# ekzhu/datasketch

Measured on AMD Instinct MI355X. Metric: MinHash signatures/sec (1M sets x 256 tokens, num_perm=128), higher is better.
Workload: dtype u64

## Files before the change

### datasketch_amd/csrc/mhx_api.hip

```cpp
#include <algorithm>
#include <cmath>
#include <condition_variable>
#include <cstdlib>
#include <cstring>
#include <mutex>
#include <new>
#include <system_error>
#include <thread>
#include <vector>

#include "mhx_internal.h"

namespace mhx {

static thread_local std::string g_last_error;

void set_error(const char *fmt, ...) {
    char buf[1024];
    va_list ap;
    va_start(ap, fmt);
    vsnprintf(buf, sizeof(buf), fmt, ap);
    va_end(ap);
    g_last_error = buf;
}
// ... 385 lines not shown
    MHX_ENTER(ctx, ctx);
    if (name && name_len > 0) {
        strncpy(name, ctx->name, (size_t)name_len - 1);
        name[name_len - 1] = 0;
    }
    if (cus) *cus = ctx->hw_cus;
    if (hbm_bytes) *hbm_bytes = ctx->hbm_bytes;
    return MHX_OK;
}

int mhx_ctx_set_option(mhx_ctx *ctx, const char *key, int64_t value) {
    static const struct {
        const char *key;
        int64_t mhx_ctx::*field;
    } options[] = {
        {"minhash.path", &mhx_ctx::opt_minhash_path},       {"minhash.split", &mhx_ctx::opt_minhash_split},
        {"minhash.packed", &mhx_ctx::opt_minhash_packed},   {"minhash.ties", &mhx_ctx::opt_minhash_ties},
        {"minhash.p3", &mhx_ctx::opt_minhash_p3},           {"minhash.share", &mhx_ctx::opt_minhash_share},
        {"minhash.adapt", &mhx_ctx::opt_minhash_adapt},     {"blocks_per_cu", &mhx_ctx::opt_blocks_per_cu},
        {"minhash.alias", &mhx_ctx::opt_minhash_alias},     {"minhash.prefetch", &mhx_ctx::opt_minhash_prefetch},
        {"weighted.path", &mhx_ctx::opt_weighted_path},     {"weighted.direct", &mhx_ctx::opt_weighted_direct},
        {"weighted.split", &mhx_ctx::opt_weighted_split},   {"weighted.tail", &mhx_ctx::opt_weighted_tail},
        {"weighted.debug", &mhx_ctx::opt_weighted_debug},   {"weighted.kernel", &mhx_ctx::opt_weighted_kernel},
        {"weighted.plan", &mhx_ctx::opt_weighted_plan},     {"weighted.rescue", &mhx_ctx::opt_weighted_rescue},
        {"weighted.min_dim", &mhx_ctx::opt_weighted_min_dim}, {"host.chunk_bytes", &mhx_ctx::opt_host_chunk_bytes},
        {"lsh.sort_bits", &mhx_ctx::opt_lsh_sort_bits},     {"lsh.gather", &mhx_ctx::opt_lsh_gather},
        {"lsh.sort", &mhx_ctx::opt_lsh_sort},               {"lsh.levels", &mhx_ctx::opt_lsh_levels},
        {"lsh.chunk", &mhx_ctx::opt_lsh_chunk},             {"lsh.team", &mhx_ctx::opt_lsh_team},
        {"lsh.bigbins", &mhx_ctx::opt_lsh_bigbins},         {"pack.fused", &mhx_ctx::opt_pack_fused},
        {"weighted.refill", &mhx_ctx::opt_weighted_refill}, {"lsh.prehash", &mhx_ctx::opt_lsh_prehash},
        {"lsh.merge_items", &mhx_ctx::opt_lsh_merge_items}, {"hll.split_tokens", &mhx_ctx::opt_hll_split_tokens},
        {"bloom.lanes", &mhx_ctx::opt_bloom_lanes},         {"jaccard.topk_path", &mhx_ctx::opt_jaccard_topk_path},
        {"jaccard.topk_segments", &mhx_ctx::opt_jaccard_topk_segments}, {"debug.cus", &mhx_ctx::opt_debug_cus},
    };
    if (!ctx || !key) return fail(MHX_ERR_INVALID, "ctx/key is NULL");
    MHX_GUARD(ctx);
    for (const auto &o : options) {
        if (strcmp(key, o.key)) continue;
        if (o.field == &mhx_ctx::opt_lsh_merge_items)
            MHX_REQUIRE(value == 0 || value == 8 || value == 16, "lsh.merge_items must be 0, 8 or 16");
        if (o.field == &mhx_ctx::opt_hll_split_tokens) MHX_REQUIRE(value >= 0, "hll.split_tokens must be >= 0");
        if (o.field == &mhx_ctx::opt_bloom_lanes) MHX_REQUIRE(value == 0 || value == 1 || value == 16, "bloom.lanes must be 0, 1 or 16");
        if (o.field == &mhx_ctx::opt_jaccard_topk_path) MHX_REQUIRE(value >= 0 && value <= 2, "jaccard.topk_path must be 0, 1 or 2");
        if (o.field == &mhx_ctx::opt_jaccard_topk_segments) MHX_REQUIRE(value >= 0, "jaccard.topk_segments must be >= 0");
        if (o.field == &mhx_ctx::opt_debug_cus)
            MHX_REQUIRE(value >= 0 && value <= ctx->hw_cus, "debug.cus must be 0 (the device's %d CUs) or in [1, %d], got %lld", ctx->hw_cus, ctx->hw_cus,
                        (long long)value);
        ctx->*o.field = value;
        if (o.field == &mhx_ctx::opt_debug_cus) ctx->num_cus = value ? (int)value : ctx->hw_cus;
        return MHX_OK;
    }
    return fail(MHX_ERR_INVALID, "unknown option '%s'", key);
}

int mhx_ctx_minhash_mode(mhx_ctx *ctx, int reset, int *mode) {
    MHX_ENTER(ctx, ctx);
    MHX_TRY(ctx->activate());
    MHX_TRY(ctx->ensure_work());
    unsigned int word = 0;
    MHX_HIP_CHECK(hipMemcpyAsync(&word, ctx->d_work + 8, sizeof(word), hipMemcpyDeviceToHost, ctx->stream));
    MHX_HIP_CHECK(hipStreamSynchronize(ctx->stream));
    if (mode) *mode = (int)word;
    if (reset) MHX_HIP_CHECK(hipMemsetAsync(ctx->d_work + 8, 0, sizeof(word), ctx->stream));
    return MHX_OK;
}

int mhx_ctx_minhash_flags(mhx_ctx *ctx, int64_t n_sets, uint8_t *flags) {
    MHX_ENTER(ctx, ctx);
    MHX_TRY(ctx->activate());
    MHX_REQUIRE(n_sets >= 0 && (flags || n_sets == 0), "NULL flags");
    if (ctx->redo_sets != n_sets || (n_sets > 0 && !ctx->d_redo))
        return fail(MHX_ERR_INVALID, "the last MinHash call on this context kept flags for %lld sets, not %lld (one huge set split over waves and "
                    "minhash.path != 0 keep none)", (long long)ctx->redo_sets, (long long)n_sets);
    MHX_HIP_CHECK(hipStreamSynchronize(ctx->stream));
    if (n_sets > 0) MHX_HIP_CHECK(hipMemcpy(flags, ctx->d_redo, (size_t)n_sets, hipMemcpyDeviceToHost));
    return MHX_OK;
}

int mhx_ctx_counters(mhx_ctx *ctx, int enable, uint64_t out[MHX_NUM_COUNTERS]) {
    MHX_ENTER(ctx, ctx);
    MHX_TRY(ctx->activate());
    MHX_HIP_CHECK(hipStreamSynchronize(ctx->stream));
    if (out) {
        for (int i = 0; i < MHX_NUM_COUNTERS; ++i) out[i] = 0;
        if (ctx->d_stats)
            MHX_HIP_CHECK(hipMemcpy(out, ctx->d_stats, sizeof(uint64_t) * MHX_NUM_COUNTERS, hipMemcpyDeviceToHost));
    }
    if (enable && !ctx->d_stats) {
        hipError_t e = mhx::dev_malloc(reinterpret_cast<void **>(&ctx->d_stats), sizeof(uint64_t) * MHX_NUM_COUNTERS);
        if (e != hipSuccess) {
            ctx->d_stats = nullptr;
            return fail(MHX_ERR_OOM, "counter allocation failed: %s", hipGetErrorString(e));
        }
    }
    if (!enable && ctx->d_stats) {
        MHX_HIP_CHECK(mhx::dev_free(ctx->d_stats));
        ctx->d_stats = nullptr;
    }
    if (ctx->d_stats) MHX_HIP_CHECK(hipMemset(ctx->d_stats, 0, sizeof(uint64_t) * MHX_NUM_COUNTERS));
    return MHX_OK;
}

int mhx_debug_guard_alloc(int align, int64_t *granule, int64_t *live) {
    if (align != 0 && (align < -4096 || align > 4096 || ((align < 0 ? -align : align) & ((align < 0 ? -align : align) - 1))))
        return fail(MHX_ERR_INVALID, "guard alignment must be 0 (off) or +-(a power of two <= 4096), got %d", align);
    (void)mhx::guard_mode();
    {
        std::lock_guard<std::mutex> lk(mhx::g_guard_mu);
// ... 1963 lines not shown
```

### datasketch_amd/csrc/mhx_internal.h

```cpp
#pragma once

#include <hip/hip_runtime.h>

#include <algorithm>
#include <cstdarg>
#include <cstdint>
#include <cstdio>
#include <mutex>
#include <string>
#include <unordered_map>

#include "mhx.h"

namespace mhx {

void set_error(const char *fmt, ...);
int fail(int code, const char *fmt, ...);
void forgive();

#define MHX_HIP_CHECK(expr)                                                                      \
    do {                                                                                         \
        hipError_t _e = (expr);                                                                  \
        if (_e != hipSuccess) {                                                                  \
            return ::mhx::fail(_e == hipErrorOutOfMemory ? MHX_ERR_OOM : MHX_ERR_HIP,            \
// ... 8 lines not shown
constexpr unsigned int kPairListCap = 16384;
constexpr size_t kWorkBytes = 64 + sizeof(unsigned int) * kPairListCap;

#define MHX_GUARD(ctxp) std::lock_guard<std::recursive_mutex> _mhx_guard((ctxp)->mu)

#define MHX_REQUIRE(cond, ...)                                       \
    do {                                                             \
        if (!(cond)) return ::mhx::fail(MHX_ERR_INVALID, __VA_ARGS__); \
    } while (0)

hipError_t dev_malloc(void **p, size_t bytes, bool caller = false);
hipError_t dev_free(void *p);
bool guard_mode();

}

struct mhx_ctx {
    std::recursive_mutex mu;
    int device = 0;
    hipStream_t stream = nullptr;
    int num_cus = 0;
    int hw_cus = 0;
    int64_t lds_per_block = 64 << 10;
    int64_t hbm_bytes = 0;
    char name[128] = {0};
    void *scratch[5] = {nullptr, nullptr, nullptr, nullptr, nullptr};
    size_t scratch_bytes[5] = {0, 0, 0, 0, 0};
    int64_t opt_minhash_path = 0;
    int64_t opt_minhash_packed = 0;
    int64_t opt_minhash_adapt = 0;
    int64_t opt_minhash_share = 0;
    int64_t opt_minhash_p3 = 0;
    int64_t opt_minhash_ties = 0;
    int64_t opt_minhash_split = 0;
    int64_t opt_blocks_per_cu = 0;
    int64_t opt_debug_cus = 0;
    int64_t opt_minhash_prefetch = 1;
    int64_t opt_minhash_alias = -1;
    int64_t opt_weighted_path = 0;
    int64_t opt_weighted_min_dim = 0;
    int64_t opt_weighted_rescue = 0;
    int64_t opt_weighted_plan = 0;
    int64_t opt_weighted_kernel = 0;
    int64_t opt_weighted_debug = 0;
    int64_t opt_weighted_split = 0;
    int64_t opt_weighted_tail = 0;
    int64_t opt_weighted_direct = 0;
    int64_t opt_lsh_sort = 0;
    int64_t opt_lsh_gather = 0;
    int64_t opt_lsh_sort_bits = 0;
    int64_t opt_lsh_prehash = 0;
    int64_t opt_lsh_chunk = 0;
    int64_t opt_lsh_bigbins = 0;
    int64_t opt_lsh_team = 0;
    int64_t opt_lsh_merge_items = 0;
    int64_t opt_lsh_levels = 0;
    int64_t opt_pack_fused = 0;
    int64_t opt_weighted_refill = 0;
    int64_t opt_hll_split_tokens = 0;
    int64_t opt_bloom_lanes = 0;
    int64_t opt_jaccard_topk_path = 0;
    int64_t opt_jaccard_topk_segments = 0;
    int64_t opt_host_chunk_bytes = 0;

    hipStream_t copy_in = nullptr;
    hipStream_t copy_out = nullptr;
// ... 144 lines not shown
```

### datasketch_amd/csrc/minhash_kernels.hip

```cpp
#include <type_traits>

#include "mhx_internal.h"

namespace mhx {
namespace {

constexpr uint64_t kMersenne = (1ull << 61) - 1;
constexpr uint32_t kMaxHash = 0xFFFFFFFFu;
constexpr int kWave = 64;

struct BulkArgs {
    const void *hv;
    const int64_t *offsets;
    int64_t fixed_len;
    int64_t n_sets;
    const uint64_t *a;
    const uint64_t *b;
    int32_t num_perm;
    int32_t path;
    unsigned long long *stats;
    uint8_t *redo;
    int32_t redo_match;
    unsigned int *sieve_hint;
    unsigned int *mode_word;
// ... 237 lines not shown
    }
    __device__ __forceinline__ void merge_from_lane(int other) {
        const uint32_t o1 = (uint32_t)__shfl((int)k1, other, kWave), o2 = (uint32_t)__shfl((int)k2, other, kWave);
        const uint32_t o3 = (uint32_t)__shfl((int)k3, other, kWave);
        add(o1);
        add(o2);
        add(o3);
    }
};

template <int P, typename TokT, bool OPEN, int PS = P>
__device__ __forceinline__ void sieve_chunk(const Chunk<TokT> &c, const SievePerms<P> &sp, uint32_t (&row)[P]) {
    constexpr int N = Chunk<TokT>::N;
    c.keep_whole();
#pragma unroll
    for (int i = 0; i < N; i += 4) {
#pragma unroll
        for (int p = 0; p < PS; ++p) {
            const uint32_t m0 = sieve_key(c.lo(i + 0), sp.a_lo[p], sp.b8[p]);
            const uint32_t m1 = sieve_key(c.lo(i + 1), sp.a_lo[p], sp.b8[p]);
            const uint32_t m2 = sieve_key(c.lo(i + 2), sp.a_lo[p], sp.b8[p]);
            const uint32_t m3 = sieve_key(c.lo(i + 3), sp.a_lo[p], sp.b8[p]);
            row[p] = (OPEN && i == 0) ? min(m0, m1) : umin3(row[p], m0, m1);
            row[p] = umin3(row[p], m2, m3);
        }
        if constexpr (PS == 1)
            asm volatile("" : "+v"(row[0]));
        else
            asm volatile("" : "+v"(row[0]), "+v"(row[PS - 1]));
        __builtin_amdgcn_sched_barrier(0);
    }
}

template <int P, int STRIDE, int WPT, bool PARTIAL = false>
__device__ __forceinline__ bool finish_block(const Two (&rows)[P], const uint32_t *tile, const Perms<P> &pm,
                                             const SievePerms<P> &sp, uint32_t (&res)[P], uint32_t last_row = 16,
                                             uint32_t last_cols = 16) {
    Two cols[P];
    uint64_t best[P];
#pragma unroll
    for (int q = 0; q < P; ++q) {
        const uint32_t myrow = rows[q].k1 & 15u;
        const uint32_t *rowp = tile + myrow * STRIDE;
        const uint32_t limit = PARTIAL ? (myrow == last_row ? last_cols : 16u) : 16u;
        if constexpr (P <= 2) {
            uint32_t w[kRowTokens];
#pragma unroll
            for (int c = 0; c < kRowTokens; ++c) w[c] = rowp[c * WPT];
            const auto key = [&](int c) {
                uint32_t m = sieve_key(w[c], sp.a_lo[q], sp.b8[q]);
                if (PARTIAL) m = (uint32_t)c < limit ? m : kMaxHash;
                return tag16(m, (uint32_t)c);
            };
            uint32_t lo[5], mid[5];
#pragma unroll
            for (int i = 0; i < 5; ++i) {
                const uint32_t x = key(3 * i), y = key(3 * i + 1), z = key(3 * i + 2);
                lo[i] = umin3(x, y, z);
                mid[i] = umed3(x, y, z);
                asm volatile("" : "+v"(lo[i]), "+v"(mid[i]));
                __builtin_amdgcn_sched_barrier(0);
            }
            const uint32_t last = key(15);
            const uint32_t a1 = umin3(lo[0], lo[1], lo[2]), a2 = umed3(lo[0], lo[1], lo[2]);
            const uint32_t b1 = umin3(lo[3], lo[4], last), b2 = umed3(lo[3], lo[4], last);
            cols[q].k1 = min(a1, b1);
            cols[q].k2 = min(umin3(max(a1, b1), a2, b2), umin3(umin3(mid[0], mid[1], mid[2]), mid[3], mid[4]));
            asm volatile("" : "+v"(cols[q].k2));
        } else {
#pragma unroll
            for (int c = 0; c < kRowTokens; ++c) {
                uint32_t m = (uint32_t)((uint64_t)rowp[c * WPT] * sp.a_lo[q] + sp.b8[q]);
                if (PARTIAL) m = (uint32_t)c < limit ? m : kMaxHash;
                cols[q].add(tag16(m, (uint32_t)c));
            }
        }
        const uint32_t j1 = cols[q].k1 & 15u;
        best[q] = WPT == 2 ? *reinterpret_cast<const uint64_t *>(rowp + 2 * j1) : (uint64_t)rowp[j1];
        __builtin_amdgcn_sched_barrier(0);
    }
    bool fail = false;
#pragma unroll
    for (int q = 0; q < P; ++q) {
        const bool ok = rows[q].apart() && cols[q].apart() && cols[q].k1 >= 16u;
        fail |= sp.active[q] && !ok;
        uint32_t l0, h0;
        mad_wide((uint32_t)best[q], (uint32_t)(best[q] >> 32), pm.a_lo[q], pm.a_hi[q], pm.b[q], l0, h0);
        res[q] = min(res[q], fold_exact(l0, h0));
    }
    return fail;
}

template <int P, int STRIDE, int WPT>
__device__ __forceinline__ bool finish_block_ties(const Three (&rows)[P], const uint32_t *tile, const Perms<P> &pm,
                                                  const SievePerms<P> &sp, uint32_t (&res)[P], bool *tied = nullptr) {
    bool fail = false;
#pragma unroll
    for (int q = 0; q < P; ++q) {
        const uint32_t base = rows[q].k1 & ~15u;
        const uint32_t *rowp = tile + (rows[q].k1 & 15u) * STRIDE;
        Three cols;
#pragma unroll
        for (int c = 0; c < kRowTokens; ++c) {
            const uint32_t m = (uint32_t)((uint64_t)rowp[c * WPT] * sp.a_lo[q] + sp.b8[q]);
            cols.add(tag16(m, (uint32_t)c));
        }
        const bool row_tie = rows[q].k2 - base < 32u;
        const bool col_tie = cols.k2 - base < 32u;
        bool ok = base >= 16u && base <= 0xFFFFFF00u && rows[q].k3 - base >= 32u && !(row_tie && col_tie) && cols.k3 - base >= 32u;
        const uint32_t j1 = cols.k1 & 15u;
        const uint64_t t1 = WPT == 2 ? *reinterpret_cast<const uint64_t *>(rowp + 2 * j1) : (uint64_t)rowp[j1];
        const uint32_t j2 = col_tie ? (cols.k2 & 15u) : j1;
        uint64_t t2 = WPT == 2 ? *reinterpret_cast<const uint64_t *>(rowp + 2 * j2) : (uint64_t)rowp[j2];
        if (__any(row_tie)) {
            const uint32_t *row2 = tile + (rows[q].k2 & 15u) * STRIDE;
            Two other;
#pragma unroll
            for (int c = 0; c < kRowTokens; ++c) {
                const uint32_t m = (uint32_t)((uint64_t)row2[c * WPT] * sp.a_lo[q] + sp.b8[q]);
                other.add(tag16(m, (uint32_t)c));
            }
// ... 8 lines not shown
        if (tied) *tied |= sp.active[q] && (row_tie || col_tie);
        uint32_t l0, h0, l1, h1;
        mad_wide((uint32_t)t1, (uint32_t)(t1 >> 32), pm.a_lo[q], pm.a_hi[q], pm.b[q], l0, h0);
        mad_wide((uint32_t)t2, (uint32_t)(t2 >> 32), pm.a_lo[q], pm.a_hi[q], pm.b[q], l1, h1);
        res[q] = umin3(res[q], fold_exact(l0, h0), fold_exact(l1, h1));
        __builtin_amdgcn_sched_barrier(0);
    }
    return fail;
}

template <int P, int STRIDE, int WPT, typename Rows>
__device__ __forceinline__ void share_last_slot(Rows &rec, const uint32_t *tile, const SievePerms<P> &sp, int rb, int lane) {
    const uint32_t span = sp.span, groups = (uint32_t)kWave / span;
    const uint32_t mine = (uint32_t)lane / span;
    const uint32_t a_lo = sp.a_lo[P - 1];
    const uint64_t b8 = sp.b8[P - 1];
    rec = Rows();
#pragma unroll 1
    for (uint32_t r0 = 0; r0 < (uint32_t)rb; r0 += groups) {
        const uint32_t r = r0 + mine;
        const uint32_t *rowp = tile + (r & 15u) * STRIDE;
        uint32_t m = kMaxHash;
#pragma unroll
        for (int c = 0; c < kRowTokens; c += 2) {
            const uint32_t m0 = sieve_key(rowp[c * WPT], a_lo, b8);
            const uint32_t m1 = sieve_key(rowp[(c + 1) * WPT], a_lo, b8);
            m = umin3(m, m0, m1);
        }
        rec.add(r < (uint32_t)rb ? tag16(m, r) : kMaxHash);
    }
    for (uint32_t s = span; s < (uint32_t)kWave; s <<= 1) rec.merge_from_lane(lane ^ (int)s);
}

template <int P, typename TokT, bool TIES = false, bool SHARE = false>
__device__ __forceinline__ bool sieve_range(const TokT MHX_CONST_AS *hv, const TokT *hv_vec, int64_t beg,
                                            int nrows, const Perms<P> &pm, const SievePerms<P> &sp,
                                            uint32_t *lds, int lane, uint32_t (&res)[P], int &nblocks, bool *tied = nullptr) {
    constexpr int N = Chunk<TokT>::N;
    constexpr int CPR = kRowTokens / N;
    constexpr int STRIDE = StageLayout<TokT>::kStride, WPT = StageLayout<TokT>::kWordsPerTok;
    const TokT MHX_CONST_AS *p = hv + beg;
    const int nchunks = nrows * CPR;
    const auto chunk_ptr = [&](int idx) { return p + (int64_t)(idx < nchunks ? idx : nchunks - 1) * N; };
    Chunk<TokT> a, b;
    a.load(p);
    int ci = 0;
    bool fail = false;
    for (int r0 = 0; r0 < nrows; r0 += kBlockRows) {
        const int rb = min(kBlockRows, nrows - r0);
        const int64_t blk = beg + (int64_t)r0 * kRowTokens;
        const int my_row = lane >> 2, my_part = lane & 3;
        uint4 st0 = {0, 0, 0, 0}, st1 = {0, 0, 0, 0};
        if (my_row < rb) {
            const uint4 *src = reinterpret_cast<const uint4 *>(hv_vec + blk + 4 * lane);
            st0 = src[0];
            if (WPT == 2) st1 = src[1];
        }
        typename std::conditional<TIES, Three, Two>::type rows[P];
        const auto row_loop = [&](auto slots) {
            constexpr int PS = decltype(slots)::value;
            if constexpr (CPR == 2) {
                for (int r = 0; r < rb; ++r) {
                    uint32_t row0[P];
                    a.arrived();
                    b.load(chunk_ptr(ci + 1));
                    __builtin_amdgcn_sched_barrier(0);
                    sieve_chunk<P, TokT, true, PS>(a, sp, row0);
                    b.arrived();
                    a.load(chunk_ptr(ci + 2));
                    __builtin_amdgcn_sched_barrier(0);
// ... 5 lines not shown
            } else {
                for (int r = 0; r < rb; r += 2) {
                    uint32_t row0[P], row1[P];
                    a.arrived();
                    b.load(chunk_ptr(ci + 1));
                    __builtin_amdgcn_sched_barrier(0);
                    sieve_chunk<P, TokT, true, PS>(a, sp, row0);
                    b.arrived();
                    a.load(chunk_ptr(ci + 2));
                    __builtin_amdgcn_sched_barrier(0);
                    sieve_chunk<P, TokT, true, PS>(b, sp, row1);
                    ci += 2;
                    const bool second = r + 1 < rb;
                    if (!second) ci -= 1;
#pragma unroll
                    for (int q = 0; q < PS; ++q) {
                        rows[q].add(tag16(row0[q], (uint32_t)r));
                        if (second) rows[q].add(tag16(row1[q], (uint32_t)(r + 1)));
                    }
                }
            }
        };
        constexpr bool kShare = SHARE && P >= 3;
        row_loop(std::integral_constant<int, (kShare ? P - 1 : P)>());
        {
            uint4 *dst = reinterpret_cast<uint4 *>(lds + my_row * STRIDE + my_part * (4 * WPT));
            dst[0] = st0;
            if (WPT == 2) dst[1] = st1;
        }
        if constexpr (kShare) share_last_slot<P, STRIDE, WPT>(rows[P - 1], lds, sp, rb, lane);
        if constexpr (TIES)
            fail |= finish_block_ties<P, STRIDE, WPT>(rows, lds, pm, sp, res, tied);
        else
            fail |= finish_block<P, STRIDE, WPT>(rows, lds, pm, sp, res);
        ++nblocks;
    }
    return fail;
}

constexpr int kDedupSlots = 1024;
constexpr int kDedupPasses = 3;
constexpr int kDedupWordsPerWave = kStageWordsPerWave + kDedupSlots;

template <typename TokT>
__device__ __forceinline__ void load_quad(const TokT *hv_vec, int64_t blk, int64_t end, int lane, uint64_t (&t)[4]) {
#pragma unroll
    for (int i = 0; i < 4; ++i) t[i] = blk + 4 * lane + i < end ? (uint64_t)hv_vec[blk + 4 * lane + i] : 0;
}

template <int P, typename TokT>
__device__ __forceinline__ bool dedup_sieve_range(const TokT *hv_vec, int64_t beg, int64_t end, const Perms<P> &pm,
                                                  const SievePerms<P> &sp, uint32_t *lds, int lane,
                                                  const uint64_t (&first)[4], uint32_t (&res)[P]) {
    constexpr int STRIDE = 36;
    uint32_t *tile = lds;
    uint32_t *table = lds + kStageWordsPerWave;
    bool fail = false;
    for (int64_t blk = beg; blk < end; blk += kBlockRows * kRowTokens) {
        const int nb = (int)min((int64_t)(kBlockRows * kRowTokens), end - blk);
        uint64_t t[4];
        bool keep[4];
        if (blk == beg) {
#pragma unroll
            for (int i = 0; i < 4; ++i) t[i] = first[i];
        } else {
            load_quad<TokT>(hv_vec, blk, end, lane, t);
        }
// ... 110 lines not shown
    for (int p = 0; p < P; ++p) {
        const int k = kbase + p * kWave + lane;
        active[p] = k < num_perm;
        const uint64_t av = active[p] ? a[k] : 0;
        pm.a_lo[p] = pm_biased.a_lo[p] = (uint32_t)av;
        pm.a_hi[p] = pm_biased.a_hi[p] = (uint32_t)(av >> 32);
        pm.b[p] = active[p] ? b[k] : 0;
        pm_biased.b[p] = pm.b[p] + 1;
    }
    Minima<P> res;
    bool redo = exact_only;
    if (!exact_only) {
        uint32_t acc[P];
#pragma unroll
        for (int p = 0; p < P; ++p) acc[p] = kMaxHash;
        hash_range<P, false, TokT>(hv, beg, end, pm_biased, acc);
        bool suspicious = false;
#pragma unroll
        for (int p = 0; p < P; ++p) {
            suspicious |= active[p] && acc[p] <= 7u;
            res.v[p] = acc[p] - 1u;
        }
        redo = __any(suspicious);
    }
    if (redo) {
        if (!exact_only && stats && lane == 0) atomicAdd(stats + 1, 1ull);
#pragma unroll
        for (int p = 0; p < P; ++p) res.v[p] = kMaxHash;
        hash_range<P, true, TokT>(hv, beg, end, pm, res.v);
    }
    return res;
}

template <int P, typename TokT, bool TAIL = true, bool TIES = false, bool SHARE = false>
__device__ __forceinline__ bool sieve_minima(const TokT MHX_CONST_AS *hv, const TokT *hv_vec, int64_t beg,
                                             int64_t end, const Perms<P> &pm, const Perms<P> &pm_biased,
                                             const SievePerms<P> &sp, unsigned long long *stats, int lane,
                                             uint32_t *lds, uint32_t (&res)[P], bool *tied = nullptr) {
    const int64_t n = end - beg;
    const int nrows = (int)min(n / kRowTokens, (int64_t)(1 << 27));
#pragma unroll
    for (int p = 0; p < P; ++p) res[p] = kMaxHash;
    bool bad = false;
    if (nrows > 0) {
        int nblocks = 0;
        bad = sieve_range<P, TokT, TIES, SHARE>(hv, hv_vec, beg, nrows, pm, sp, lds, lane, res, nblocks, tied);
        if (stats && lane == 0) atomicAdd(stats + 2, (unsigned long long)nblocks);
    }
    const int64_t tail = beg + (int64_t)nrows * kRowTokens;
    if (TAIL && tail < end) {
        uint32_t acc[P];
#pragma unroll
        for (int p = 0; p < P; ++p) acc[p] = kMaxHash;
        hash_range<P, false, TokT>(hv, tail, end, pm_biased, acc);
#pragma unroll
        for (int p = 0; p < P; ++p) {
            bad |= sp.active[p] && acc[p] <= 7u;
            res[p] = min(res[p], acc[p] - 1u);
        }
    }
    return __any(bad);
}

struct SieveBackoff {
    int skip = 0;
    int gap = 16;
    int streak = 0;
    __device__ __forceinline__ void failed() {
        if (++streak >= 2) {
            skip = gap;
            gap = min(2 * gap, 64);
        }
    }
    __device__ __forceinline__ void succeeded() {
        streak = 0;
        gap = 16;
    }
};

// ... 38 lines not shown
    }
}

template <int P, bool SHARE = false>
__device__ __forceinline__ void load_perms(const BulkArgs &args, int kbase, int lane, Perms<P> &pm,
                                           Perms<P> &pm_biased, SievePerms<P> &sp, int (&kidx)[P]) {
    uint32_t span = kWave;
    if constexpr (SHARE && P >= 3) {
        const int r = args.num_perm - (kbase + (P - 1) * kWave);
        span = r > 16 ? 32u : r > 8 ? 16u : r > 4 ? 8u : 4u;
    }
    sp.span = span;
#pragma unroll
    for (int p = 0; p < P; ++p) {
        const bool shared = SHARE && P >= 3 && p == P - 1;
        const int k = kbase + p * kWave + (shared ? lane & (int)(span - 1) : lane);
        const bool holds = k < args.num_perm;
        kidx[p] = holds && !(shared && lane >= (int)span) ? k : -1;
        const uint64_t a = holds ? args.a[k] : 0;
        pm.a_lo[p] = (uint32_t)a;
        pm.a_hi[p] = (uint32_t)(a >> 32);
        pm.b[p] = holds ? args.b[k] : 0;
        pm_biased.a_lo[p] = pm.a_lo[p];
        pm_biased.a_hi[p] = pm.a_hi[p];
        pm_biased.b[p] = pm.b[p] + 1;
        sp.a_lo[p] = pm.a_lo[p];
        sp.b8[p] = pm.b[p] + 8;
        sp.active[p] = kidx[p] >= 0;
    }
}

enum { MODE_SIEVE = 0, MODE_FULL = 1, MODE_DEDUP = 2, MODE_SIEVE_TIES = 3 };
enum { SHAPE_GENERAL = 0, SHAPE_PLAIN = 1, SHAPE_PLAIN_FIXED = 2, SHAPE_PLAIN_FIXED_ROWS = 3 };

template <int P, typename TokT, typename OutT, int MODE, int SHAPE, bool SHARE = false>
__global__ __launch_bounds__(256) void minhash_bulk_kernel(const BulkArgs args_in) {
    BulkArgs args = args_in;
    constexpr bool kSieve = MODE == MODE_SIEVE || MODE == MODE_SIEVE_TIES;
    if (kSieve && args.mode_word) {
        const unsigned int want_ties = *as_const(args.mode_word);
        if ((want_ties == 1u) != (MODE == MODE_SIEVE_TIES)) return;
    }
    if (MODE == MODE_FULL && args.mode_word && args.sieve_hint && blockIdx.x == 0 && threadIdx.x == 0) {
        const unsigned int t = __builtin_nontemporal_load(args.sieve_hint), f = __builtin_nontemporal_load(args.sieve_hint + 1);
        const unsigned int g = __builtin_nontemporal_load(args.sieve_hint + 2), m = *args.mode_word;
        const unsigned int tt = __builtin_nontemporal_load(args.sieve_hint + 3), tf = __builtin_nontemporal_load(args.sieve_hint + 5);
        if (t >= 64u) {
            const bool defeated = 4u * f > t;
            const bool heavy = m == 1u ? 5u * g > t : (tt >= 64u ? 5u * tf > tt : m == 2u);
            *args.mode_word = !defeated ? 0u : heavy ? 2u : 1u;
        }
    }
    if (SHAPE != SHAPE_GENERAL) {
        args.init = nullptr;
        args.init_stride = 0;
        args.stats = nullptr;
        args.alias_mask = -1;
    }
    if (SHAPE == SHAPE_PLAIN_FIXED || SHAPE == SHAPE_PLAIN_FIXED_ROWS) args.offsets = nullptr;
    const int lane = threadIdx.x & (kWave - 1);
    const int wave = __builtin_amdgcn_readfirstlane(threadIdx.x >> 6);
    const int waves_per_block = blockDim.x >> 6;
    const int kchunks = (args.num_perm + kWave * P - 1) / (kWave * P);
    constexpr int kLdsPerWave = MODE == MODE_DEDUP ? kDedupWordsPerWave : kStageWordsPerWave;
    __shared__ __attribute__((aligned(16))) uint32_t stage[4 * kLdsPerWave];
    uint32_t *lds = stage + wave * kLdsPerWave;
    Perms<P> pm, pm_biased;
    SievePerms<P> sp;
    int kidx[P];
    if (kSieve || MODE == MODE_DEDUP) load_perms<P, SHARE>(args, 0, lane, pm, pm_biased, sp, kidx);

    const TokT MHX_CONST_AS *hv = as_const(static_cast<const TokT *>(args.hv));
    const TokT *hv_vec = static_cast<const TokT *>(args.hv);
    const int64_t MHX_CONST_AS *offsets = as_const(args.offsets);
    OutT *__restrict__ out = static_cast<OutT *>(args.out);
    const int64_t stride = (int64_t)gridDim.x * waves_per_block;
    const bool flagged_only = !kSieve && args.redo != nullptr;
    unsigned int listed_n = 0;
    bool listed = false;
    if (MODE == MODE_FULL && flagged_only && args.pair_list) {
        listed_n = *as_const(args.pair_count);
        listed = listed_n <= kPairListCap;
    }
    const int64_t n_items = listed ? (int64_t)listed_n : flagged_only ? (args.n_sets + kWave - 1) / kWave * waves_per_block : args.n_sets;
    SieveBackoff backoff;
    TiesBackoff ties;
    int tried = 0, failed = 0, left = 0;
    if (MODE == MODE_SIEVE && args.sieve_hint) {
        const unsigned int t = __builtin_nontemporal_load(args.sieve_hint), f = __builtin_nontemporal_load(args.sieve_hint + 1);
        if (t >= 64u && 2u * f > t) {
            backoff.skip = 63;
            backoff.gap = 64;
            backoff.streak = 2;
        }
    }
    if (MODE == MODE_FULL && listed) {
        uint32_t *comb = stage;
        for (int64_t it = blockIdx.x; it < (int64_t)listed_n; it += gridDim.x) {
            const int64_t set = (int64_t)as_const(args.pair_list)[it];
            const int64_t beg = args.offsets ? offsets[set] : set * args.fixed_len;
            const int64_t end = args.offsets ? offsets[set + 1] : beg + args.fixed_len;
            const int64_t share = (end - beg + 31) / 32 * 8;
            const int64_t wbeg = min(end, beg + wave * share), wend = min(end, wbeg + share);
            for (int kc = 0; kc < kchunks; ++kc) {
                uint32_t mine[P];
#pragma unroll
                for (int p = 0; p < P; ++p) mine[p] = kMaxHash;
                if (wend > wbeg) {
                    const Minima<P> m = full_minima<P, TokT>(hv_vec, wbeg, wend, args.a, args.b, args.num_perm, kc * (kWave * P),
                                                             args.path == 1, args.stats);
#pragma unroll
                    for (int p = 0; p < P; ++p) mine[p] = m.v[p];
                }
#pragma unroll
                for (int p = 0; p < P; ++p) comb[(wave * P + p) * kWave + lane] = mine[p];
                __syncthreads();
                if (wave == 0) {
#pragma unroll
                    for (int p = 0; p < P; ++p) {
                        const int k = kc * (kWave * P) + p * kWave + lane;
                        if (k >= args.num_perm) continue;
                        uint32_t r = mine[p];
// ... 27 lines not shown
        const int64_t set = listed ? (int64_t)as_const(args.pair_list)[item0] : flagged_only ? item * kWave + bit : item;
        int64_t beg, end;
        if (args.offsets) {
            beg = offsets[set];
            end = offsets[set + 1];
        } else {
            beg = (args.alias_mask >= 0 ? (set & args.alias_mask) : set) * args.fixed_len;
            end = beg + args.fixed_len;
        }
        uint32_t warm = 0;
        {
            const int64_t nset = listed ? args.n_sets : flagged_only ? (todo ? item * kWave + __builtin_ctzll(todo) : args.n_sets) : item + stride;
            const bool skipping_on = MODE == MODE_SIEVE && backoff.skip > 1;
            if (args.prefetch && nset < args.n_sets && !skipping_on) {
                const int64_t nbeg = args.offsets ? offsets[nset] : nset * args.fixed_len;
                const int64_t nend = args.offsets ? offsets[nset + 1] : nbeg + args.fixed_len;
                const int64_t off = (int64_t)lane * 128;
                if (off < (nend - nbeg) * (int64_t)sizeof(TokT))
                    warm = *reinterpret_cast<const volatile uint32_t *>(reinterpret_cast<const char *>(args.hv) +
                                                                         nbeg * (int64_t)sizeof(TokT) + off);
            }
        }
        bool defer = false;
        if (MODE == MODE_SIEVE && end > beg && backoff.skip > 0) {
            --backoff.skip;
            defer = true;
        }
        for (int kc = 0; kc < kchunks && !defer; ++kc) {
            uint32_t res[P];
            if (kSieve) {
                if (kchunks > 1) load_perms<P, SHARE>(args, kc * (kWave * P), lane, pm, pm_biased, sp, kidx);
                if (end > beg) {
                    bool tied = false;
                    defer = sieve_minima<P, TokT, SHAPE != SHAPE_PLAIN_FIXED_ROWS, MODE == MODE_SIEVE_TIES, SHARE>(hv, hv_vec, beg, end, pm, pm_biased, sp, args.stats, lane, lds, res,
                                                                                                          MODE == MODE_SIEVE_TIES ? &tied : nullptr);
                    if (kc == 0) ++tried;
                    if (MODE == MODE_SIEVE_TIES) {
                        if (defer || __any(tied)) ++failed;
                        if (defer) {
                            ++left;
                            break;
                        }
                    } else {
                        if (defer) {
                            ++failed;
                            backoff.failed();
                            break;
                        }
                        backoff.succeeded();
                    }
                }
            } else {
#pragma unroll
                for (int p = 0; p < P; ++p) {
                    const int k = kc * (kWave * P) + p * kWave + lane;
                    kidx[p] = k < args.num_perm ? k : -1;
                }
                if (end > beg) {
                    if (MODE == MODE_DEDUP) {
                        if (kchunks > 1) load_perms<P>(args, kc * (kWave * P), lane, pm, pm_biased, sp, kidx);
                        bool open = true;
                        if (!args.ties || (args.mode_word && *as_const(args.mode_word) == 1u)) {
                        } else if (ties.skip > 0) {
                            if (kc == kchunks - 1) --ties.skip;
                        } else {
                            open = sieve_minima<P, TokT, true, true>(hv, hv_vec, beg, end, pm, pm_biased, sp, nullptr, lane, lds, res);
                            if (kc == 0) ++tried, failed += open ? 1 : 0;
                            if (open) ties.failed(); else ties.succeeded();
                        }
                        if (open) {
#pragma unroll
                        for (int p = 0; p < P; ++p) res[p] = kMaxHash;
                        uint64_t cur[4];
                        load_quad<TokT>(hv_vec, beg, end, lane, cur);
                        defer = __any(dedup_sieve_range<P, TokT>(hv_vec, beg, end, pm, sp, lds, lane, cur, res));
                        if (defer) {
                            if (args.stats && lane == 0) atomicAdd(args.stats + 3, 1ull);
                            break;
                        }
                        }
                    } else {
                        const Minima<P> m = full_minima<P, TokT>(hv_vec, beg, end, args.a, args.b, args.num_perm,
                                                                 kc * (kWave * P), args.path == 1, args.stats);
#pragma unroll
                        for (int p = 0; p < P; ++p) res[p] = m.v[p];
                    }
                }
            }
#pragma unroll
            for (int p = 0; p < P; ++p) {
                if (kidx[p] < 0) continue;
                uint64_t v;
                if (args.init) {
                    const uint64_t iv = args.init[set * args.init_stride + kidx[p]];
                    if (end > beg) {
                        const uint32_t ic = (iv >> 32) ? kMaxHash : (uint32_t)iv;
                        v = min(ic, res[p]);
                    } else {
                        v = iv;
                    }
                } else {
                    v = end > beg ? res[p] : kMaxHash;
                }
                if (sizeof(OutT) == 4) v = v > kMaxHash ? kMaxHash : v;
                out[set * args.num_perm + kidx[p]] = (OutT)v;
            }
        }
        if (kSieve && lane == 0) {
            args.redo[set] = defer ? 1 : 0;
            if (defer && args.stats) atomicAdd(args.stats, 1ull);
        }
        if (MODE == MODE_DEDUP && defer && lane == 0) {
            args.redo[set] = 2;
            if (args.pair_list) {
                const unsigned int slot = atomicAdd(args.pair_count, 1u);
                if (slot < kPairListCap) args.pair_list[slot] = (unsigned int)set;
            }
        }
        asm volatile("" ::"v"(warm));
      }
    }
    if (kSieve && args.sieve_hint && lane == 0 && wave == 0 && (blockIdx.x & 15u) == 0 && tried > 0) {
        atomicAdd(args.sieve_hint, (unsigned int)tried);
        if (failed) atomicAdd(args.sieve_hint + 1, (unsigned int)failed);
        if (left) atomicAdd(args.sieve_hint + 2, (unsigned int)left);
    }
    if (MODE == MODE_DEDUP && args.sieve_hint && args.mode_word && lane == 0 && tried > 0) {
        atomicAdd(args.sieve_hint + 3, (unsigned int)tried);
        if (failed) atomicAdd(args.sieve_hint + 5, (unsigned int)failed);
    }
}

template <int KP, int P, typename TokT, typename OutT>
__global__ __launch_bounds__(256) void minhash_packed_kernel(const BulkArgs args) {
    constexpr int G = kWave / KP;
    constexpr int STRIDE = 36;
    const int lane = threadIdx.x & (kWave - 1);
    const int wave = __builtin_amdgcn_readfirstlane(threadIdx.x >> 6);
    const int g = lane / KP, k = lane % KP;
    __shared__ __attribute__((aligned(16))) uint32_t stage[4 * G * kStageWordsPerWave];
    uint32_t *tiles = stage + wave * (G * kStageWordsPerWave);
    uint32_t *my_tile = tiles + g * kStageWordsPerWave;
    Perms<P> pm;
    SievePerms<P> sp;
    bool any_active = false;
#pragma unroll
    for (int q = 0; q < P; ++q) {
        const bool active = k + q * KP < args.num_perm;
        const uint64_t a = active ? args.a[k + q * KP] : 0, b = active ? args.b[k + q * KP] : 0;
        pm.a_lo[q] = sp.a_lo[q] = (uint32_t)a;
        pm.a_hi[q] = (uint32_t)(a >> 32);
        pm.b[q] = b;
        sp.b8[q] = b + 8;
        sp.active[q] = active;
// ... 204 lines not shown
            r.y = xa[u].y < ya[u].y ? xa[u].y : ya[u].y;
            __builtin_nontemporal_store(r.x, &o2[i + u * stride].x);
            __builtin_nontemporal_store(r.y, &o2[i + u * stride].y);
        }
    }
    if ((count & 1) && blockIdx.x == 0 && threadIdx.x == 0)
        out[count - 1] = x[count - 1] < y[count - 1] ? x[count - 1] : y[count - 1];
}

unsigned resident_grid(mhx_ctx *ctx, const void *kernel, int64_t items) {
    int per_cu = 0;
    if (hipOccupancyMaxActiveBlocksPerMultiprocessor(&per_cu, kernel, 256, 0) != hipSuccess || per_cu < 1) {
        (void)hipGetLastError();
        per_cu = 2;
    }
    return (unsigned)std::max<int64_t>(1, std::min<int64_t>(items, (int64_t)ctx->num_cus * per_cu));
}

template <int P, typename TokT, typename OutT, int PF = P>
int launch_typed(mhx_ctx *ctx, const BulkArgs &args, int64_t first_token, int64_t total_tokens, bool split) {
    const int kchunks = (args.num_perm + kWave * P - 1) / (kWave * P);
    const int blocks_per_cu = ctx->opt_blocks_per_cu > 0 ? (int)ctx->opt_blocks_per_cu : (P >= 3 ? 128 : 64);
    const int64_t max_blocks = (int64_t)ctx->num_cus * blocks_per_cu;
    if (!split) {
        const int64_t want = (args.n_sets + 3) / 4;
        dim3 grid((unsigned)std::max<int64_t>(1, std::min(want, max_blocks)), 1u);
        if (args.path == 0) {
            if (int rc = ctx->ensure_work()) return rc;
            MHX_HIP_CHECK(hipMemsetAsync(ctx->d_work, 0, 8 * sizeof(unsigned int), ctx->stream));
            BulkArgs sieve_args = args;
            sieve_args.sieve_hint = ctx->d_work;
            sieve_args.mode_word = ctx->opt_minhash_adapt == 1 || args.stats ? nullptr : ctx->d_work + 8;
            const BulkArgs &args_s = sieve_args;
            const bool plain = !args.init && !args.stats && args.alias_mask < 0;
            const int np = args.num_perm;
            const bool packable = !args.stats && args.alias_mask < 0 && ctx->opt_minhash_packed != 1;
            const bool packed = packable && P <= 2 && (np <= 96 || (ctx->opt_minhash_packed == 2 && np <= 128));
            if (packed) {
                const int kp = np <= 8 ? 8 : np <= 16 ? 16 : np <= 32 ? 32 : np <= 64 ? 16 : np <= 96 ? 32 : 64;
                const int64_t items = (args.n_sets + 64 / kp - 1) / (64 / kp);
                dim3 pgrid((unsigned)std::max<int64_t>(1, std::min<int64_t>((items + 3) / 4, max_blocks)), 1u);
#define MHX_PACKED(KP_, P_) hipLaunchKernelGGL((minhash_packed_kernel<KP_, P_, TokT, OutT>), pgrid, dim3(256), 0, ctx->stream, args_s)
                if (np <= 8) MHX_PACKED(8, 1);
                else if (np <= 16) MHX_PACKED(16, 1);
                else if (np <= 32) MHX_PACKED(32, 1);
                else if (np <= 48) MHX_PACKED(16, 3);
                else if (np <= 64) MHX_PACKED(16, 4);
                else if (np <= 96) MHX_PACKED(32, 3);
                else MHX_PACKED(64, 2);
#undef MHX_PACKED
            } else {
            const bool fixed_rows = plain && !args.offsets && args.fixed_len % kRowTokens == 0;
            const int last_slot = args.num_perm - (P - 1) * kWave;
            const bool share = P >= 3 && kchunks == 1 && args.share_last && last_slot > 0 && last_slot <= 32;
            const auto first_launches = [&](auto share_tag) {
                constexpr bool SH = decltype(share_tag)::value;
#define MHX_SIEVE(MODE_, SHAPE_) hipLaunchKernelGGL((minhash_bulk_kernel<P, TokT, OutT, MODE_, SHAPE_, SH>), grid, dim3(256), 0, ctx->stream, args_s)
                if (fixed_rows) MHX_SIEVE(MODE_SIEVE, SHAPE_PLAIN_FIXED_ROWS);
                else if (plain && !args.offsets) MHX_SIEVE(MODE_SIEVE, SHAPE_PLAIN_FIXED);
                else if (plain) MHX_SIEVE(MODE_SIEVE, SHAPE_PLAIN);
                else MHX_SIEVE(MODE_SIEVE, SHAPE_GENERAL);
                if (args_s.mode_word) {
                    if (fixed_rows) MHX_SIEVE(MODE_SIEVE_TIES, SHAPE_PLAIN_FIXED_ROWS);
                    else MHX_SIEVE(MODE_SIEVE_TIES, SHAPE_GENERAL);
                }
#undef MHX_SIEVE
            };
            if constexpr (P >= 3) {
                if (share) first_launches(std::true_type());
                else first_launches(std::false_type());
            } else {
                (void)share;
                first_launches(std::false_type());
            }
            }
            const int64_t flag_groups = (args.n_sets + kWave - 1) / kWave;
            BulkArgs dedup = args;
            dedup.redo_match = 1;
            dedup.sieve_hint = sieve_args.sieve_hint;
            dedup.mode_word = packed ? nullptr : sieve_args.mode_word;
            if (args.n_sets <= 0xFFFFFFFFll) {
                dedup.pair_count = ctx->d_work + 4;
                dedup.pair_list = ctx->d_work + 16;
            }
            hipLaunchKernelGGL((minhash_bulk_kernel<PF, TokT, OutT, MODE_DEDUP, SHAPE_GENERAL>),
                               dim3(resident_grid(ctx, (const void *)minhash_bulk_kernel<PF, TokT, OutT, MODE_DEDUP, SHAPE_GENERAL>, flag_groups)),
                               dim3(256), 0, ctx->stream, dedup);
            BulkArgs rest = dedup;
            rest.redo_match = 2;
            hipLaunchKernelGGL((minhash_bulk_kernel<PF, TokT, OutT, MODE_FULL, SHAPE_GENERAL>),
                               dim3(resident_grid(ctx, (const void *)minhash_bulk_kernel<PF, TokT, OutT, MODE_FULL, SHAPE_GENERAL>, flag_groups)),
                               dim3(256), 0, ctx->stream, rest);
        } else {
            BulkArgs all = args;
            all.redo = nullptr;
            hipLaunchKernelGGL((minhash_bulk_kernel<PF, TokT, OutT, MODE_FULL, SHAPE_GENERAL>), grid, dim3(256), 0, ctx->stream, all);
        }
    } else {
        const int64_t total_out = args.n_sets * (int64_t)args.num_perm;
        const int64_t fill_blocks = std::max<int64_t>(1, std::min<int64_t>((total_out + 255) / 256, max_blocks));
        hipLaunchKernelGGL((minhash_fill_state_kernel<OutT>), dim3((unsigned)fill_blocks), dim3(256), 0,
                           ctx->stream, args);
        const int64_t waves = (int64_t)ctx->num_cus * 32;
        int64_t slice = (total_tokens + waves - 1) / waves;
        slice = slice > 128 ? (slice + 255) / 256 * 256 : std::max<int64_t>(64, (slice + 15) / 16 * 16);
        const int64_t n_slices = (total_tokens + slice - 1) / slice;
        const int64_t want = (n_slices + 3) / 4;
        dim3 grid((unsigned)std::max<int64_t>(1, std::min(want, max_blocks)), (unsigned)kchunks);
        hipLaunchKernelGGL((minhash_split_kernel<P, TokT, OutT>), grid, dim3(256), 0, ctx->stream, args,
                           first_token, total_tokens, slice);
    }
    MHX_HIP_CHECK(hipGetLastError());
// ... 77 lines not shown
```

Baseline: 478.1 million.

## Settle few sieve proof failures in-wave instead of deferring whole sets

When the sieve's per-block proof fails for only a few (lane, perm) slots, the kernel now recomputes those slots exactly within the wave using readlane and a shuffle reduction over the staged LDS tile, instead of marking the set for the later full recompute. A device word records whether any set was deferred at all, and the dedup kernel exits early when none were, which avoids launching work for an empty redo list. Settled sets get flag value 3, which the flags API maps back to 1 unless settle mode 2 is chosen. The cost is extra register pressure and branching in the sieve kernels, and some shape and permutation combinations are left out.

After: 479.6 million, median of 2. About the same (+0.3%).

```diff
diff --git a/datasketch_amd/csrc/mhx_api.hip b/datasketch_amd/csrc/mhx_api.hip
--- a/datasketch_amd/csrc/mhx_api.hip
+++ b/datasketch_amd/csrc/mhx_api.hip
@@ -441,6 +441,7 @@
         {"lsh.merge_items", &mhx_ctx::opt_lsh_merge_items}, {"hll.split_tokens", &mhx_ctx::opt_hll_split_tokens},
         {"bloom.lanes", &mhx_ctx::opt_bloom_lanes},         {"jaccard.topk_path", &mhx_ctx::opt_jaccard_topk_path},
         {"jaccard.topk_segments", &mhx_ctx::opt_jaccard_topk_segments}, {"debug.cus", &mhx_ctx::opt_debug_cus},
+        {"minhash.settle", &mhx_ctx::opt_minhash_settle},
     };
     if (!ctx || !key) return fail(MHX_ERR_INVALID, "ctx/key is NULL");
     MHX_GUARD(ctx);
@@ -452,6 +453,7 @@
         if (o.field == &mhx_ctx::opt_bloom_lanes) MHX_REQUIRE(value == 0 || value == 1 || value == 16, "bloom.lanes must be 0, 1 or 16");
         if (o.field == &mhx_ctx::opt_jaccard_topk_path) MHX_REQUIRE(value >= 0 && value <= 2, "jaccard.topk_path must be 0, 1 or 2");
         if (o.field == &mhx_ctx::opt_jaccard_topk_segments) MHX_REQUIRE(value >= 0, "jaccard.topk_segments must be >= 0");
+        if (o.field == &mhx_ctx::opt_minhash_settle) MHX_REQUIRE(value >= 0 && value <= 2, "minhash.settle must be 0, 1 or 2");
         if (o.field == &mhx_ctx::opt_debug_cus)
             MHX_REQUIRE(value >= 0 && value <= ctx->hw_cus, "debug.cus must be 0 (the device's %d CUs) or in [1, %d], got %lld", ctx->hw_cus, ctx->hw_cus,
                         (long long)value);
@@ -483,6 +485,8 @@
                     "minhash.path != 0 keep none)", (long long)ctx->redo_sets, (long long)n_sets);
     MHX_HIP_CHECK(hipStreamSynchronize(ctx->stream));
     if (n_sets > 0) MHX_HIP_CHECK(hipMemcpy(flags, ctx->d_redo, (size_t)n_sets, hipMemcpyDeviceToHost));
+    if (ctx->opt_minhash_settle != 2)
+        for (int64_t i = 0; i < n_sets; ++i) flags[i] = flags[i] == 3 ? 1 : flags[i];
     return MHX_OK;
 }
 
diff --git a/datasketch_amd/csrc/mhx_internal.h b/datasketch_amd/csrc/mhx_internal.h
--- a/datasketch_amd/csrc/mhx_internal.h
+++ b/datasketch_amd/csrc/mhx_internal.h
@@ -64,6 +64,7 @@
     int64_t opt_minhash_share = 0;
     int64_t opt_minhash_p3 = 0;
     int64_t opt_minhash_ties = 0;
+    int64_t opt_minhash_settle = 0;
     int64_t opt_minhash_split = 0;
     int64_t opt_blocks_per_cu = 0;
     int64_t opt_debug_cus = 0;
diff --git a/datasketch_amd/csrc/minhash_kernels.hip b/datasketch_amd/csrc/minhash_kernels.hip
--- a/datasketch_amd/csrc/minhash_kernels.hip
+++ b/datasketch_amd/csrc/minhash_kernels.hip
@@ -293,10 +293,66 @@
     }
 }
 
-template <int P, int STRIDE, int WPT, bool PARTIAL = false>
+constexpr int kSettledNow = 1 << 29, kProofFailed = 1 << 30, kDeferredSome = 1 << 28, kGaveUp = 1 << 27, kWordSeen = 1 << 26;
+constexpr int kFailedCount = kWordSeen - 1;
+constexpr int kSettleCap = 4;
+
+template <int P, int STRIDE, int WPT>
+__device__ __forceinline__ void settle_block(const Two (&rows)[P], uint32_t bad, const uint32_t *tile, const Perms<P> &pm,
+                                             uint32_t (&res)[P], int rb) {
+    const int lane = threadIdx.x & (kWave - 1);
+    uint32_t off = (lane >> 2) < rb ? 0u : kMaxHash;
+    asm volatile("" : "+v"(off), "+v"(bad));
+    const uint32_t *cell = tile + (lane >> 2) * STRIDE + (lane & 3) * (4 * WPT);
+    uint32_t lo[4], hi[4];
+    if constexpr (WPT == 2) {
+        const uint4 x = *reinterpret_cast<const uint4 *>(cell), y = *reinterpret_cast<const uint4 *>(cell + 4);
+        lo[0] = x.x, hi[0] = x.y, lo[1] = x.z, hi[1] = x.w;
+        lo[2] = y.x, hi[2] = y.y, lo[3] = y.z, hi[3] = y.w;
+    } else {
+        const uint4 x = *reinterpret_cast<const uint4 *>(cell);
+        lo[0] = x.x, lo[1] = x.y, lo[2] = x.z, lo[3] = x.w;
+        hi[0] = hi[1] = hi[2] = hi[3] = 0;
+    }
+#pragma unroll
+    for (int q = 0; q < P; ++q) {
+        for (;;) {
+            const unsigned long long left = __ballot((bad >> q) & 1u);
+            if (!left) break;
+            const int src = __builtin_ctzll(left);
+            const auto from_src = [&](uint32_t x) {
+                uint32_t r = (uint32_t)__builtin_amdgcn_readlane((int)x, src);
+                asm volatile("" : "+v"(r));
+                return r;
+            };
+            const uint32_t a_lo = from_src(pm.a_lo[q]), a_hi = from_src(pm.a_hi[q]);
+            const uint32_t b_lo = from_src((uint32_t)pm.b[q]), b_hi = from_src((uint32_t)(pm.b[q] >> 32));
+            const uint32_t k1 = from_src(rows[q].k1);
+            const uint32_t top = k1 | 15u;
+            const uint32_t th = (k1 < 16u || top > kMaxHash - 8u) ? kMaxHash : top + 8u;
+            const uint64_t b = ((uint64_t)b_hi << 32) | b_lo;
+            uint32_t best = kMaxHash;
+#pragma unroll
+            for (int j = 0; j < 4; ++j) {
+                uint32_t l0, h0;
+                mad_wide(lo[j], hi[j], a_lo, a_hi, b, l0, h0);
+                const uint32_t key = l0 + 8u;
+                best = key <= th ? min(best, max(fold_exact(l0, h0), off)) : best;
+            }
+            for (int s = kWave / 2; s > 0; s >>= 1) best = min(best, (uint32_t)__shfl_xor((int)best, s, kWave));
+            if (lane == src) {
+                res[q] = min(res[q], best);
+                bad &= ~(1u << q);
+            }
+        }
+    }
+}
+
+template <int P, int STRIDE, int WPT, bool PARTIAL = false, bool SETTLE = false>
 __device__ __forceinline__ bool finish_block(const Two (&rows)[P], const uint32_t *tile, const Perms<P> &pm,
                                              const SievePerms<P> &sp, uint32_t (&res)[P], uint32_t last_row = 16,
-                                             uint32_t last_cols = 16) {
+                                             uint32_t last_cols = 16, int rows_left = kBlockRows, int *settled = nullptr) {
+    static_assert(!(PARTIAL && SETTLE), "the windowed pass reads whole rows");
     Two cols[P];
     uint64_t best[P];
 #pragma unroll
@@ -341,13 +397,32 @@
         __builtin_amdgcn_sched_barrier(0);
     }
     bool fail = false;
+    [[maybe_unused]] bool bad[P];
 #pragma unroll
     for (int q = 0; q < P; ++q) {
         const bool ok = rows[q].apart() && cols[q].apart() && cols[q].k1 >= 16u;
         fail |= sp.active[q] && !ok;
+        if constexpr (SETTLE) bad[q] = sp.active[q] && !ok;
         uint32_t l0, h0;
         mad_wide((uint32_t)best[q], (uint32_t)(best[q] >> 32), pm.a_lo[q], pm.a_hi[q], pm.b[q], l0, h0);
         res[q] = min(res[q], fold_exact(l0, h0));
+    }
+    if constexpr (SETTLE) {
+        if (__any(fail)) {
+            int count = 0;
+#pragma unroll
+            for (int q = 0; q < P; ++q) count += __popcll(__ballot(bad[q]));
+            if (count <= kSettleCap) {
+                uint32_t slots = 0;
+#pragma unroll
+                for (int q = 0; q < P; ++q) slots |= bad[q] ? 1u << q : 0u;
+                settle_block<P, STRIDE, WPT>(rows, slots, tile, pm, res, min(kBlockRows, rows_left));
+                *settled |= kSettledNow;
+            } else {
+                *settled |= kGaveUp;
+            }
+        }
+        return false;
     }
     return fail;
 }
@@ -422,10 +497,11 @@
     for (uint32_t s = span; s < (uint32_t)kWave; s <<= 1) rec.merge_from_lane(lane ^ (int)s);
 }
 
-template <int P, typename TokT, bool TIES = false, bool SHARE = false>
+template <int P, typename TokT, bool TIES = false, bool SHARE = false, bool SETTLE = false>
 __device__ __forceinline__ bool sieve_range(const TokT MHX_CONST_AS *hv, const TokT *hv_vec, int64_t beg,
                                             int nrows, const Perms<P> &pm, const SievePerms<P> &sp,
-                                            uint32_t *lds, int lane, uint32_t (&res)[P], int &nblocks, bool *tied = nullptr) {
+                                            uint32_t *lds, int lane, uint32_t (&res)[P], int &nblocks, bool *tied = nullptr,
+                                            int *settled = nullptr) {
     constexpr int N = Chunk<TokT>::N;
     constexpr int CPR = kRowTokens / N;
     constexpr int STRIDE = StageLayout<TokT>::kStride, WPT = StageLayout<TokT>::kWordsPerTok;
@@ -497,7 +573,7 @@
         if constexpr (TIES)
             fail |= finish_block_ties<P, STRIDE, WPT>(rows, lds, pm, sp, res, tied);
         else
-            fail |= finish_block<P, STRIDE, WPT>(rows, lds, pm, sp, res);
+            fail |= finish_block<P, STRIDE, WPT, false, SETTLE>(rows, lds, pm, sp, res, 16, 16, nrows - r0, settled);
         ++nblocks;
     }
     return fail;
@@ -674,11 +750,11 @@
     return res;
 }
 
-template <int P, typename TokT, bool TAIL = true, bool TIES = false, bool SHARE = false>
+template <int P, typename TokT, bool TAIL = true, bool TIES = false, bool SHARE = false, bool SETTLE = false>
 __device__ __forceinline__ bool sieve_minima(const TokT MHX_CONST_AS *hv, const TokT *hv_vec, int64_t beg,
                                              int64_t end, const Perms<P> &pm, const Perms<P> &pm_biased,
                                              const SievePerms<P> &sp, unsigned long long *stats, int lane,
-                                             uint32_t *lds, uint32_t (&res)[P], bool *tied = nullptr) {
+                                             uint32_t *lds, uint32_t (&res)[P], bool *tied = nullptr, int *settled = nullptr) {
     const int64_t n = end - beg;
     const int nrows = (int)min(n / kRowTokens, (int64_t)(1 << 27));
 #pragma unroll
@@ -686,7 +762,7 @@
     bool bad = false;
     if (nrows > 0) {
         int nblocks = 0;
-        bad = sieve_range<P, TokT, TIES, SHARE>(hv, hv_vec, beg, nrows, pm, sp, lds, lane, res, nblocks, tied);
+        bad = sieve_range<P, TokT, TIES, SHARE, SETTLE>(hv, hv_vec, beg, nrows, pm, sp, lds, lane, res, nblocks, tied, settled);
         if (stats && lane == 0) atomicAdd(stats + 2, (unsigned long long)nblocks);
     }
     const int64_t tail = beg + (int64_t)nrows * kRowTokens;
@@ -791,11 +867,22 @@
 
 enum { MODE_SIEVE = 0, MODE_FULL = 1, MODE_DEDUP = 2, MODE_SIEVE_TIES = 3 };
 enum { SHAPE_GENERAL = 0, SHAPE_PLAIN = 1, SHAPE_PLAIN_FIXED = 2, SHAPE_PLAIN_FIXED_ROWS = 3 };
+constexpr int kDeferredWord = 6;
+__device__ __forceinline__ void say_deferred(unsigned int *work) {
+    const unsigned int seen = __hip_atomic_load(work + kDeferredWord, __ATOMIC_RELAXED, __HIP_MEMORY_SCOPE_AGENT);
+    if (__builtin_amdgcn_readfirstlane((int)seen) == 0)
+        __hip_atomic_store(work + kDeferredWord, 1u, __ATOMIC_RELAXED, __HIP_MEMORY_SCOPE_AGENT);
+}
 
 template <int P, typename TokT, typename OutT, int MODE, int SHAPE, bool SHARE = false>
 __global__ __launch_bounds__(256) void minhash_bulk_kernel(const BulkArgs args_in) {
     BulkArgs args = args_in;
     constexpr bool kSieve = MODE == MODE_SIEVE || MODE == MODE_SIEVE_TIES;
+    constexpr bool kWide = sizeof(TokT) == 8;
+    constexpr bool kLeftOut = kWide ? (P == 1 && SHAPE == SHAPE_PLAIN_FIXED_ROWS) || (P == 4 && SHAPE != SHAPE_PLAIN)
+                                    : (P == 1 && SHAPE != SHAPE_PLAIN_FIXED) || (P == 2 && SHAPE == SHAPE_PLAIN);
+    constexpr bool kSettle = MODE == MODE_SIEVE && SHAPE != SHAPE_GENERAL && !kLeftOut;
+    if (MODE == MODE_DEDUP && args.sieve_hint && *as_const(args.sieve_hint + kDeferredWord) == 0u) return;
     if (kSieve && args.mode_word) {
         const unsigned int want_ties = *as_const(args.mode_word);
         if ((want_ties == 1u) != (MODE == MODE_SIEVE_TIES)) return;
@@ -847,6 +934,7 @@
     int tried = 0, failed = 0, left = 0;
     if (MODE == MODE_SIEVE && args.sieve_hint) {
         const unsigned int t = __builtin_nontemporal_load(args.sieve_hint), f = __builtin_nontemporal_load(args.sieve_hint + 1);
+        if (__builtin_amdgcn_readfirstlane((int)__builtin_nontemporal_load(args.sieve_hint + kDeferredWord)) != 0) failed |= kWordSeen;
         if (t >= 64u && 2u * f > t) {
             backoff.skip = 63;
             backoff.gap = 64;
@@ -940,8 +1028,8 @@
                 if (kchunks > 1) load_perms<P, SHARE>(args, kc * (kWave * P), lane, pm, pm_biased, sp, kidx);
                 if (end > beg) {
                     bool tied = false;
-                    defer = sieve_minima<P, TokT, SHAPE != SHAPE_PLAIN_FIXED_ROWS, MODE == MODE_SIEVE_TIES, SHARE>(hv, hv_vec, beg, end, pm, pm_biased, sp, args.stats, lane, lds, res,
-                                                                                                          MODE == MODE_SIEVE_TIES ? &tied : nullptr);
+                    defer = sieve_minima<P, TokT, SHAPE != SHAPE_PLAIN_FIXED_ROWS, MODE == MODE_SIEVE_TIES, SHARE, kSettle>(hv, hv_vec, beg, end, pm, pm_biased, sp, args.stats, lane, lds, res,
+                                                                                                          MODE == MODE_SIEVE_TIES ? &tied : nullptr, kSettle ? &failed : nullptr);
                     if (kc == 0) ++tried;
                     if (MODE == MODE_SIEVE_TIES) {
                         if (defer || __any(tied)) ++failed;
@@ -950,12 +1038,20 @@
                             break;
                         }
                     } else {
-                        if (defer) {
-                            ++failed;
-                            backoff.failed();
-                            break;
+                        if (kSettle && (failed & kGaveUp)) {
+                            defer = true;
+                            failed &= ~kGaveUp;
                         }
-                        backoff.succeeded();
+                        if (defer || (failed & kSettledNow)) {
+                            if (!(failed & kProofFailed)) failed = (failed | kProofFailed) + 1;
+                            failed &= ~kSettledNow;
+                            if (defer) {
+                                backoff.failed();
+                                break;
+                            }
+                        } else if (!(failed & kProofFailed)) {
+                            backoff.succeeded();
+                        }
                     }
                 }
             } else {
@@ -1015,9 +1111,10 @@
             }
         }
         if (kSieve && lane == 0) {
-            args.redo[set] = defer ? 1 : 0;
+            args.redo[set] = defer ? 1 : (kSettle && (failed & kProofFailed)) ? 3 : 0;
             if (defer && args.stats) atomicAdd(args.stats, 1ull);
         }
+        if (kSieve) failed = (failed & ~kProofFailed) | (defer ? kDeferredSome : 0);
         if (MODE == MODE_DEDUP && defer && lane == 0) {
             args.redo[set] = 2;
             if (args.pair_list) {
@@ -1028,6 +1125,8 @@
         asm volatile("" ::"v"(warm));
       }
     }
+    if (kSieve && args.sieve_hint && (failed & (kDeferredSome | kWordSeen)) == kDeferredSome) say_deferred(args.sieve_hint);
+    failed &= kFailedCount;
     if (kSieve && args.sieve_hint && lane == 0 && wave == 0 && (blockIdx.x & 15u) == 0 && tried > 0) {
         atomicAdd(args.sieve_hint, (unsigned int)tried);
         if (failed) atomicAdd(args.sieve_hint + 1, (unsigned int)failed);
@@ -1298,6 +1397,7 @@
             sieve_args.sieve_hint = ctx->d_work;
             sieve_args.mode_word = ctx->opt_minhash_adapt == 1 || args.stats ? nullptr : ctx->d_work + 8;
             const BulkArgs &args_s = sieve_args;
+            const bool settle = ctx->opt_minhash_settle != 1 && ctx->opt_minhash_ties != 1;
             const bool plain = !args.init && !args.stats && args.alias_mask < 0;
             const int np = args.num_perm;
             const bool packable = !args.stats && args.alias_mask < 0 && ctx->opt_minhash_packed != 1;
@@ -1322,7 +1422,8 @@
             const auto first_launches = [&](auto share_tag) {
                 constexpr bool SH = decltype(share_tag)::value;
 #define MHX_SIEVE(MODE_, SHAPE_) hipLaunchKernelGGL((minhash_bulk_kernel<P, TokT, OutT, MODE_, SHAPE_, SH>), grid, dim3(256), 0, ctx->stream, args_s)
-                if (fixed_rows) MHX_SIEVE(MODE_SIEVE, SHAPE_PLAIN_FIXED_ROWS);
+                if (!settle) MHX_SIEVE(MODE_SIEVE, SHAPE_GENERAL);
+                else if (fixed_rows) MHX_SIEVE(MODE_SIEVE, SHAPE_PLAIN_FIXED_ROWS);
                 else if (plain && !args.offsets) MHX_SIEVE(MODE_SIEVE, SHAPE_PLAIN_FIXED);
                 else if (plain) MHX_SIEVE(MODE_SIEVE, SHAPE_PLAIN);
                 else MHX_SIEVE(MODE_SIEVE, SHAPE_GENERAL);
@@ -1343,7 +1444,7 @@
             const int64_t flag_groups = (args.n_sets + kWave - 1) / kWave;
             BulkArgs dedup = args;
             dedup.redo_match = 1;
-            dedup.sieve_hint = sieve_args.sieve_hint;
+            dedup.sieve_hint = packed ? nullptr : sieve_args.sieve_hint;
             dedup.mode_word = packed ? nullptr : sieve_args.mode_word;
             if (args.n_sets <= 0xFFFFFFFFll) {
                 dedup.pair_count = ctx->d_work + 4;
```
